# leggedrobotics/delora

Measured on AMD Instinct MI355X. Metric: training scan-pairs/sec, KITTI 64x2048 range images, higher is better.
Workload: dtype f32; 1 GPU; KITTI-shaped 64x2048, batch=8 pairs/GPU, raw scans of ~141k points (ragged, raster order), steps rotate over 8 distinct HBM-resident batches, online normals, ResNet pose CNN (11.9M params, identity-pretrained state), Adam; BASELINE configs[1]; global_batch=8, parallelism=dp1, cnn=fp32, cnn_impl=hip trunk: fp32 MFMA, fused Winograd F(2x2,3x3) + direct implicit GEMM, channels_last=False, hip_graph=False, distinct_batches=8, priming_steps=8

## Files before the change

delora_amd/_lib.py:

```python
import ctypes
import os

_HERE = os.path.dirname(os.path.abspath(__file__))
LIB_PATH = os.path.join(_HERE, "csrc", "libdelora_hip.so")
ABI_VERSION = 10


class DeloraHipError(RuntimeError):
    pass


class SensorStruct(ctypes.Structure):
    _fields_ = [("H", ctypes.c_int32), ("W", ctypes.c_int32),
                ("hfov0", ctypes.c_double), ("hfov1", ctypes.c_double),
                ("vfov0", ctypes.c_double), ("vfov1", ctypes.c_double)]


class RecordLayout(ctypes.Structure):
    _fields_ = [("point_step", ctypes.c_int32), ("off_x", ctypes.c_int32), ("off_y", ctypes.c_int32), ("off_z", ctypes.c_int32),
                ("filter", ctypes.c_uint32), ("min_range", ctypes.c_float)]


RECORDS_DROP_ZERO, RECORDS_MIN_RANGE = 1, 2

# ... 48 lines not shown
    "dl_tower_conv3x3_nhwc_f32": (_i32, [_vp, _vp, _vp, _vp, _i32, _i32, _i32, _i32, _i32, _vp, _vp, _vp, _i32, _i32, _u32, _vp]),
    "dl_tower_wgrad_workspace_bytes": (_sz, [_i32, _i32, _i32, _i32, _i32]),
    "dl_tower_wgrad3x3_nhwc_f32": (_i32, [_vp, _vp, _vp, _vp, _i32, _i32, _i32, _i32, _i32, _vp, _vp, _vp]),
    "dl_narrow_conv2d_nhwc_f32": (_i32, [_vp, _vp, _vp, _vp, _vp, _i32, _i32, _i32, _i32, _i32, _i32, _i32, _i32, _i32, _i32, _u32, _vp]),
    "dl_narrow_dgrad_strided_nhwc_f32": (_i32, [_vp, _vp, _vp, _vp, _vp, _i32, _i32, _i32, _i32, _i32, _i32, _i32, _i32, _i32, _i32, _u32, _vp]),
    "dl_narrow_wgrad_workspace_bytes": (_sz, [_i32, _i32, _i32, _i32, _i32, _i32, _i32, _i32]),
    "dl_narrow_wgrad_nhwc_f32": (_i32, [_vp, _vp, _vp, _vp, _i32, _i32, _i32, _i32, _i32, _i32, _i32, _i32, _vp]),
    "dl_wino_weights_floats": (_sz, [_i32, _i32]),
    "dl_wino_weights_f32": (_i32, [_vp, _vp, _vp, _i32, _i32, _vp]),
    "dl_wino_weights_batch_f32": (_i32, [_vp, _i32, _vp]),
    "dl_wino_conv3x3_workspace_bytes": (_sz, [_i32, _i32, _i32, _i32, _i32]),
    "dl_wino_conv3x3_nhwc_f32": (_i32, [_vp, _vp, _vp, _vp, _vp, _i32, _i32, _i32, _i32, _i32, _i32, _u32, _vp, _vp]),
    "dl_wino_strided_takes": (_i32, [_i32, _i32, _i32, _i32, _i32, _i32, _i32, _i32]),
    "dl_wino_strided_weights_floats": (_sz, [_i32, _i32, _i32, _i32]),
    "dl_wino_strided_weights_f32": (_i32, [_vp, _vp, _vp, _i32, _i32, _i32, _i32, _vp]),
    "dl_wino_strided_conv3x3_nhwc_f32": (_i32, [_vp, _vp, _vp, _i32, _i32, _i32, _i32, _i32, _i32, _i32, _i32, _u32, _vp]),
    "dl_wino_strided_dgrad3x3_nhwc_f32": (_i32, [_vp, _vp, _vp, _vp, _vp, _i32, _i32, _i32, _i32, _i32, _i32, _i32, _i32, _u32, _vp]),
    "dl_wino_wgrad_workspace_bytes": (_sz, [_i32, _i32, _i32, _i32, _i32]),
    "dl_wino_wgrad3x3_nhwc_f32": (_i32, [_vp, _vp, _vp, _vp, _i32, _i32, _i32, _i32, _i32, _vp]),
    "dl_pool3x3s12_nhwc_fwd": (_i32, [_vp, _i32, _i32, _i32, _i32, _vp, _vp, _vp]),
    "dl_pool3x3s12_nhwc_bwd": (_i32, [_vp, _vp, _vp, _i32, _i32, _i32, _i32, _i32, _vp, _vp]),
    "dl_stem_wgrad_workspace_bytes": (_sz, [_i32, _i32, _i32]),
    "dl_stem_wgrad_f32": (_i32, [_vp, _vp, _vp, _vp, _i32, _i32, _i32, _i32, _vp, _vp, _vp]),
    "dl_quat_to_T_fwd": (_i32, [_vp, _vp, _i32, ctypes.c_float, _vp, _vp]),
    "dl_quat_to_T_bwd": (_i32, [_vp, _vp, _i32, ctypes.c_float, _vp, _vp, _vp]),
    "dl_mean_hw_nhwc_f32": (_i32, [_vp, _i32, _i32, _i32, _vp, _vp]),
    "dl_conv_weights_h": (_i32, [_vp, _vp, _vp, _i32, _i32, _i32, _i32, _vp]),
    "dl_conv_weights_batch_h": (_i32, [_vp, _i32, _i32, _vp]),
    "dl_conv2d_nhwc_h": (_i32, [_vp, _vp, _vp, _vp, _vp, _i32, _i32, _i32, _i32, _i32, _i32, _i32, _i32, _i32, _i32, _i32, _u32, _vp]),
    "dl_conv2d_dgrad_strided_nhwc_h": (_i32, [_vp, _vp, _vp, _vp, _vp, _i32, _i32, _i32, _i32, _i32, _i32, _i32, _i32, _i32, _i32, _i32,
                                              _u32, _vp, _vp]),
    "dl_cast_f32_to_h": (_i32, [_vp, _vp, _i64, _i32, _vp]),
    "dl_heads_fwd": (_i32, [_vp, _vp, _i32, _i32, _i32, _i32, _i32, _vp, _vp, _vp, _vp, _vp, _vp, _vp]),
    "dl_heads_bwd_workspace_bytes": (_sz, [_i32, _i32, _i32, _i32]),
    "dl_heads_bwd": (_i32, [_vp, _vp, _i32, _i32, _i32, _i32, _i32, _vp, _vp, _vp, _vp, _vp, _vp, _vp, _vp, _vp, _vp]),
    "dl_heads_fwd_drop": (_i32, [_vp, _vp, _i32, _i32, _i32, _i32, _i32, _vp, _vp, _vp, _vp, _vp, _vp, _vp, _vp]),
    "dl_heads_bwd_drop": (_i32, [_vp, _vp, _i32, _i32, _i32, _i32, _i32, _vp, _vp, _vp, _vp, _vp, _vp, _vp, _vp, _vp, _vp, _vp]),
    "dl_heads_single_fwd": (_i32, [_vp, _vp, _i32, _i32, _i32, _i32, _i32, _i32, _i32, _i32, _vp, _vp, _vp, _vp, _vp, _vp, _vp]),
    "dl_heads_single_bwd_workspace_bytes": (_sz, [_i32, _i32, _i32, _i32, _i32, _i32, _i32]),
    "dl_heads_single_bwd": (_i32, [_vp, _vp, _i32, _i32, _i32, _i32, _i32, _i32, _i32, _i32, _vp, _vp, _vp, _vp, _vp, _vp, _vp, _vp, _vp, _vp]),
    "dl_dropout_scale_f32": (_i32, [_vp, _u32, ctypes.c_double, _i64, _vp, _vp]),
    "dl_stem_input_nhwc_drop_f32": (_i32, [_vp, _i32, _i32, _i32, _i32, _vp, ctypes.c_double, _vp, _vp]),
    "dl_channel_scale_nhwc_t": (_i32, [_vp, _vp, _i32, _i32, _i32, _i32, _vp, _vp]),
    "dl_channel_scale_bwd_act_nhwc_t": (_i32, [_vp, _vp, _vp, _i32, _i32, _i32, _i32, _i32, _vp, _vp]),
    "dl_tower_wide_drop_f32": (_i32, [_vp, _vp, ctypes.c_double, _i32, _i32, _i32, _i32, _i32, _vp, _vp]),
    "dl_tower_wide_drop_bwd_f32": (_i32, [_vp, _vp, _vp, ctypes.c_double, _i32, _i32, _i32, _i32, _i32, _i32, _vp, _vp]),
# ... 135 lines not shown
```

delora_amd/csrc/infer.hip:

```cpp
#include <stdint.h>
#include <stdio.h>
#include <string.h>

#include "common.h"

typedef uint32_t u32x4i __attribute__((ext_vector_type(4)));

__global__ __launch_bounds__(DL_BLOCK) void k_interleave_pair(const uint32_t* __restrict__ prev, size_t prev_ss, const uint32_t* __restrict__ cur,
                                                              size_t cur_ss, uint32_t HW, uint32_t total, u32x4i* __restrict__ x8) {
  const uint32_t i = blockIdx.x * DL_BLOCK + threadIdx.x;
  if (i >= total) return;
  const uint32_t b = i / HW, p = i - b * HW;
  const uint32_t* a = prev + (size_t)b * prev_ss + p;
  const uint32_t* c = cur + (size_t)b * cur_ss + p;
  const u32x4i lo = {a[0], a[HW], a[2 * (size_t)HW], a[3 * (size_t)HW]};
  const u32x4i hi = {c[0], c[HW], c[2 * (size_t)HW], c[3 * (size_t)HW]};
  x8[2 * (size_t)i] = lo;
  x8[2 * (size_t)i + 1] = hi;
}

__global__ void k_single_scan_offsets(int32_t* __restrict__ offs, int32_t n) {
  if (threadIdx.x < 2) offs[threadIdx.x] = threadIdx.x ? n : 0;
}

// ... 97 lines not shown
}

int at_layer(const char* who, const char* what, int block, int rc) {
  if (!rc) return DL_OK;
  char inner[160];
  snprintf(inner, sizeof(inner), "%s", g_dl_err);
  if (block >= 0) return dl_fail(rc, "%s: blocks[%d].%s: %s", who, block, what, inner);
  return dl_fail(rc, "%s: %s: %s", who, what, inner);
}

int pose_forward(const char* who, const dl_pose_net* net, const PosePlan& p, const void* prepared, const float* image_prev, int64_t prev_ss,
                 const float* image_cur, int64_t cur_ss, int B, int H, int W, void* workspace, float* translation, float* quaternion, float* T,
                 dl_stream stream) {
  char* const ws = (char*)workspace;
  float* slot[4];
  for (int i = 0; i < 4; ++i) slot[i] = (float*)(ws + p.slot_off[i]);
  void* const split_ws = p.split_bytes ? (void*)(ws + p.split_off) : nullptr;
  const int act = net->act;
  hipStream_t st = (hipStream_t)stream;
  const uint32_t total = (uint32_t)B * H * W;
  hipLaunchKernelGGL(k_interleave_pair, dim3((total + DL_BLOCK - 1) / DL_BLOCK), dim3(DL_BLOCK), 0, st, (const uint32_t*)image_prev, (size_t)prev_ss,
                     (const uint32_t*)image_cur, (size_t)cur_ss, (uint32_t)(H * W), total, (u32x4i*)slot[0]);
  if (int rc = dl_check_launch(who)) return rc;
  if (int rc = at_layer(who, "conv1", -1, dl_conv2d_nhwc_f32(slot[0], net->conv1_w, slot[1], nullptr, nullptr, B, H, W, 8, 64, 3, 1, 2, 0, act, DL_CONV_ACT, stream)))
    return rc;
  if (int rc = at_layer(who, "pooling", -1, dl_pool3x3s12_nhwc_fwd(slot[1], B, H, W / 2, 64, slot[2], (int8_t*)(ws + p.win_off), stream))) return rc;
  const float* u = (const float*)prepared;
  int s = 2, h = H, w = W / 4;
  for (int i = 0; i < net->n_blocks; ++i) {
    const dl_pose_block& b = net->blocks[i];
    const int ho = ceil_div(h, b.stride_h), wo = ceil_div(w, b.stride_w);
    const float* x = slot[s];
    float *y1 = slot[(s + 1) & 3], *sc = slot[(s + 2) & 3], *y2 = slot[(s + 3) & 3];
    int rc;
    if (runs_wino(b.stride_h, b.stride_w)) {
      rc = dl_wino_conv3x3_nhwc_f32(x, u, y1, nullptr, nullptr, B, h, w, b.cin, b.cout, act, DL_CONV_ACT, split_ws, stream);
      u += dl_wino_weights_floats(b.cout, b.cin);
    } else {
      rc = dl_conv2d_nhwc_f32(x, b.w1, y1, nullptr, nullptr, B, h, w, b.cin, b.cout, 3, b.stride_h, b.stride_w, 0, act, DL_CONV_ACT, stream);
    }
    if ((rc = at_layer(who, "w1", i, rc))) return rc;
    const float* shortcut = x;
    if (b.has_downsample) {
      if ((rc = at_layer(who, "wd", i, dl_conv2d_nhwc_f32(x, b.wd, sc, nullptr, nullptr, B, h, w, b.cin, b.cout, 1, b.stride_h, b.stride_w, 0, 0, 0, stream))))
        return rc;
      shortcut = sc;
    }
// ... 139 lines not shown
```

delora_amd/csrc/stem.hip:

```cpp
#include "common.h"

#define ST_TANH 1
#define ST_RELU 2

typedef float f32x4s __attribute__((ext_vector_type(4)));

__global__ __launch_bounds__(DL_BLOCK) void k_pool_nhwc_fwd(const float* __restrict__ a, int H, int Wc, int C4, uint32_t total,
                                                            float* __restrict__ y, int8_t* __restrict__ win) {
  const uint32_t i = blockIdx.x * DL_BLOCK + threadIdx.x;
  if (i >= total) return;
  const int Wp = Wc >> 1;
  const uint32_t pix = i / (uint32_t)C4;
  const int c4 = (int)(i - pix * (uint32_t)C4);
  const uint32_t nr = pix / (uint32_t)Wp;
  const int q = (int)(pix - nr * (uint32_t)Wp);
  const int r = (int)(nr % (uint32_t)H);
  const int first = r > 0 ? 0 : 3;
  f32x4s best = {-INFINITY, -INFINITY, -INFINITY, -INFINITY};
  int k0 = first, k1 = first, k2 = first, k3 = first;
#pragma unroll
  for (int dh = -1; dh <= 1; ++dh) {
    if (r + dh < 0 || r + dh >= H) continue;
    const float* row = a + ((size_t)(nr + dh) * Wc) * (size_t)(4 * C4) + 4 * c4;
#pragma unroll
    for (int dw = -1; dw <= 1; ++dw) {
      int j = 2 * q + dw;
      j = j < 0 ? j + Wc : j;
      const f32x4s v = *reinterpret_cast<const f32x4s*>(row + (size_t)j * (4 * C4));
      const int k = (dh + 1) * 3 + dw + 1;
      if (v.x > best.x || v.x != v.x) { best.x = v.x; k0 = k; }
      if (v.y > best.y || v.y != v.y) { best.y = v.y; k1 = k; }
      if (v.z > best.z || v.z != v.z) { best.z = v.z; k2 = k; }
      if (v.w > best.w || v.w != v.w) { best.w = v.w; k3 = k; }
    }
  }
  *reinterpret_cast<f32x4s*>(y + (size_t)i * 4) = best;
  *reinterpret_cast<uint32_t*>(win + (size_t)i * 4) = (uint32_t)k0 | ((uint32_t)k1 << 8) | ((uint32_t)k2 << 16) | ((uint32_t)k3 << 24);
}

__device__ __forceinline__ f32x4s pool_bwd_value(const float* __restrict__ g, const float* __restrict__ a, const int8_t* __restrict__ win,
                                                 int H, int Wc, int C4, int act, uint32_t nr, int r, int j, int c4) {
  const int Wp = Wc >> 1;
  const int q0 = j >> 1, col0 = 1 + (j & 1);
  const int q1 = (q0 + 1 == Wp) ? 0 : q0 + 1;
  const bool two = (j & 1) != 0;
  uint32_t w4[6];
  f32x4s gv[6];
  uint32_t code[6];
#pragma unroll
  for (int d = -1; d <= 1; ++d) {
    const bool row_ok = r + d >= 0 && r + d < H;
    const size_t rowbase = (size_t)(nr + (row_ok ? d : 0)) * Wp;
#pragma unroll
    for (int t = 0; t < 2; ++t) {
      const int i = (d + 1) * 2 + t;
      const size_t e = ((rowbase + ((t && two) ? q1 : q0)) * (size_t)C4 + c4) * 4;
      w4[i] = *reinterpret_cast<const uint32_t*>(win + e);
      gv[i] = *reinterpret_cast<const f32x4s*>(g + e);
      code[i] = (row_ok && (t == 0 || two)) ? (uint32_t)((1 - d) * 3 + (t ? 0 : col0)) : 0xffu;
    }
  }
  f32x4s acc = {0.f, 0.f, 0.f, 0.f};
#pragma unroll
  for (int i = 0; i < 6; ++i) {
    acc.x += (w4[i] & 0xffu) == code[i] ? gv[i].x : 0.f;
    acc.y += ((w4[i] >> 8) & 0xffu) == code[i] ? gv[i].y : 0.f;
    acc.z += ((w4[i] >> 16) & 0xffu) == code[i] ? gv[i].z : 0.f;
    acc.w += (w4[i] >> 24) == code[i] ? gv[i].w : 0.f;
  }
  const f32x4s av = *reinterpret_cast<const f32x4s*>(a + (((size_t)nr * Wc + j) * C4 + c4) * 4);
  f32x4s out;
  if (act == ST_TANH) {
    out.x = acc.x * (1.f - av.x * av.x); out.y = acc.y * (1.f - av.y * av.y);
    out.z = acc.z * (1.f - av.z * av.z); out.w = acc.w * (1.f - av.w * av.w);
  } else if (act == ST_RELU) {
    out.x = av.x <= 0.f ? 0.f : acc.x; out.y = av.y <= 0.f ? 0.f : acc.y;
    out.z = av.z <= 0.f ? 0.f : acc.z; out.w = av.w <= 0.f ? 0.f : acc.w;
  } else {
    out = acc;
  }
  return out;
}

__global__ __launch_bounds__(DL_BLOCK) void k_pool_nhwc_bwd(const float* __restrict__ g, const float* __restrict__ a,
                                                            const int8_t* __restrict__ win, int H, int Wc, int C4, int act,
                                                            uint32_t total, float* __restrict__ g_conv) {
  const uint32_t i = blockIdx.x * DL_BLOCK + threadIdx.x;
  if (i >= total) return;
  const uint32_t pix = i / (uint32_t)C4;
  const int c4 = (int)(i - pix * (uint32_t)C4);
  const uint32_t nr = pix / (uint32_t)Wc;
  const int j = (int)(pix - nr * (uint32_t)Wc);
  const int r = (int)(nr % (uint32_t)H);
  *reinterpret_cast<f32x4s*>(g_conv + (size_t)i * 4) = pool_bwd_value(g, a, win, H, Wc, C4, act, nr, r, j, c4);
}

#define SG_PX 64
#define SG_XCOLS (2 * SG_PX + 2)
typedef float f32x16s __attribute__((ext_vector_type(16)));

__global__ __launch_bounds__(DL_BLOCK, 2) void k_stem_wgrad(const float* __restrict__ g, const float* __restrict__ a,
                                                            const int8_t* __restrict__ win, const float* __restrict__ x8, int N, int H,
                                                            int Wc, int act, int chunks_per_slab, float* __restrict__ part) {
  constexpr int K = 64, C4 = 16;
  __shared__ __attribute__((aligned(16))) float gc[SG_PX * K];
  __shared__ __attribute__((aligned(16))) float xt[3 * SG_XCOLS * 8];
  const int tid = threadIdx.x, lane = tid & 63, wave = tid >> 6;
  const int li = lane & 31, half = lane >> 5;
  const int W = 2 * Wc;
  const int cpr = (Wc + SG_PX - 1) / SG_PX;
  const int total = N * H * cpr;
  const int ch_begin = blockIdx.x * chunks_per_slab, ch_end = min(ch_begin + chunks_per_slab, total);
  f32x16s acc[2][3];
#pragma unroll
  for (int i = 0; i < 2; ++i)
#pragma unroll
    for (int j = 0; j < 3; ++j)
#pragma unroll
      for (int r = 0; r < 16; ++r) acc[i][j][r] = 0.f;
  int b_off[3];
#pragma unroll
  for (int ns = 0; ns < 3; ++ns) {
    const int j = min(li + 32 * ns, 71), tap = j >> 3, c = j & 7;
    b_off[ns] = ((tap / 3) * SG_XCOLS + (tap % 3)) * 8 + c;
  }
  for (int ch = ch_begin; ch < ch_end; ++ch) {
    const int cb = ch % cpr;
    const uint32_t nr = (uint32_t)(ch / cpr);
    const int h = (int)(nr % (uint32_t)H), wc0 = cb * SG_PX;
    __syncthreads();
#pragma unroll
    for (int it = 0; it < SG_PX * C4 / DL_BLOCK; ++it) {
      const int q = tid + it * DL_BLOCK, pl = q / C4, c4 = q % C4;
      f32x4s v = {0.f, 0.f, 0.f, 0.f};
      if (wc0 + pl < Wc) v = pool_bwd_value(g, a, win, H, Wc, C4, act, nr, h, wc0 + pl, c4);
      *reinterpret_cast<f32x4s*>(gc + pl * K + c4 * 4) = v;
    }
    for (int q = tid; q < 3 * SG_XCOLS * 2; q += DL_BLOCK) {
      const int hp = q & 1, col = (q >> 1) % SG_XCOLS, row = (q >> 1) / SG_XCOLS;
      const int hh = h + row - 1;
      int w = (2 * wc0 - 1 + col) % W;
      w = w < 0 ? w + W : w;
      f32x4s v = {0.f, 0.f, 0.f, 0.f};
      if (hh >= 0 && hh < H) v = *reinterpret_cast<const f32x4s*>(x8 + (((size_t)(nr + row - 1)) * W + w) * 8 + hp * 4);
      *reinterpret_cast<f32x4s*>(xt + (row * SG_XCOLS + col) * 8 + hp * 4) = v;
    }
    __syncthreads();
#pragma unroll
    for (int ks = 0; ks < 8; ++ks) {
      const int pl = wave * 16 + ks * 2 + half;
      const float a0 = gc[pl * K + li], a1 = gc[pl * K + 32 + li];
      float b[3];
#pragma unroll
      for (int ns = 0; ns < 3; ++ns) b[ns] = xt[b_off[ns] + 2 * pl * 8];
#pragma unroll
      for (int ns = 0; ns < 3; ++ns) {
        acc[0][ns] = __builtin_amdgcn_mfma_f32_32x32x2f32(a0, b[ns], acc[0][ns], 0, 0, 0);
        acc[1][ns] = __builtin_amdgcn_mfma_f32_32x32x2f32(a1, b[ns], acc[1][ns], 0, 0, 0);
      }
    }
  }
  __syncthreads();
  float* red = gc;
#pragma unroll
  for (int ms = 0; ms < 2; ++ms)
#pragma unroll
    for (int ns = 0; ns < 3; ++ns) {
      if (wave > 0)
#pragma unroll
        for (int r = 0; r < 16; ++r) red[(wave - 1) * 1024 + r * 64 + lane] = acc[ms][ns][r];
      __syncthreads();
      if (wave == 0) {
#pragma unroll
        for (int r = 0; r < 16; ++r) acc[ms][ns][r] = ((acc[ms][ns][r] + red[r * 64 + lane]) + red[1024 + r * 64 + lane]) + red[2048 + r * 64 + lane];
        const int j = ns * 32 + li;
        if (j < 72)
#pragma unroll
          for (int r = 0; r < 16; ++r) {
            const int k = ms * 32 + (r & 3) + 8 * (r >> 2) + 4 * half;
            part[((size_t)blockIdx.x * K + k) * 72 + j] = acc[ms][ns][r];
          }
      }
      __syncthreads();
    }
}

__global__ __launch_bounds__(DL_BLOCK) void k_stem_wgrad_reduce(const float* __restrict__ part, int nslabs, float* __restrict__ dw) {
  __shared__ float red[4][64];
  const int i = blockIdx.x * 64 + (threadIdx.x & 63), w = threadIdx.x >> 6;
  float s = 0.f;
  int sl = w;
  for (; sl + 28 < nslabs; sl += 32) {
    float v[8];
#pragma unroll
    for (int u = 0; u < 8; ++u) v[u] = part[(size_t)(sl + 4 * u) * 64 * 72 + i];
#pragma unroll
    for (int u = 0; u < 8; ++u) s += v[u];
  }
  for (; sl < nslabs; sl += 4) s += part[(size_t)sl * 64 * 72 + i];
  red[w][threadIdx.x & 63] = s;
  __syncthreads();
  if (w == 0) {
    const float t = ((red[0][threadIdx.x] + red[1][threadIdx.x]) + red[2][threadIdx.x]) + red[3][threadIdx.x];
// ... 61 lines not shown

static int stem_wgrad_slabs(int total_chunks) { return total_chunks < 512 ? total_chunks : 512; }

extern "C" size_t dl_stem_wgrad_workspace_bytes(int32_t N, int32_t H, int32_t W) {
  if (N <= 0 || H <= 0 || W <= 0 || W % 4) return 0;
  return (size_t)stem_wgrad_slabs(N * H * ((W / 2 + SG_PX - 1) / SG_PX)) * 64 * 72 * sizeof(float);
}

extern "C" int dl_stem_wgrad_f32(const float* g_pooled, const float* a, const int8_t* win, const float* x8, int32_t N, int32_t H,
                                 int32_t W, int32_t act, void* workspace, float* dw, dl_stream stream) {
  if (!g_pooled || !a || !win || !x8 || !workspace || !dw || N <= 0 || H <= 0 || W <= 0 || act < 0 || act > 2)
    return dl_fail(DL_ERR_INVALID_ARGUMENT, "dl_stem_wgrad_f32: bad argument");
  if (W % 4 || (size_t)N * H * W * 32 >= ((size_t)1 << 32))
    return dl_fail(DL_ERR_UNSUPPORTED, "dl_stem_wgrad_f32: N=%d H=%d W=%d not supported (W %% 4, conv1 output below 2^32 elements)", N, H, W);
  const int Wc = W / 2, total = N * H * ((Wc + SG_PX - 1) / SG_PX), nslabs = stem_wgrad_slabs(total);
  const int cps = (total + nslabs - 1) / nslabs, grid = (total + cps - 1) / cps;
  hipStream_t st = (hipStream_t)stream;
  const DlProfTag tag{"k_stem_wgrad", "wgrad", N, H, W, 8, 64, 3, 1, 2, 2.0 * N * H * Wc * 64.0 * 72.0,
                      4.0 * ((double)N * H * Wc * 64 * 1.5 + (double)N * H * W * 8) + (double)N * H * (Wc / 2) * 64};
  DL_LAUNCH(tag, k_stem_wgrad, dim3(grid), dim3(DL_BLOCK), st, g_pooled, a, win, x8, N, H, Wc, act, cps, (float*)workspace);
  hipLaunchKernelGGL(k_stem_wgrad_reduce, dim3(64 * 72 / 64), dim3(DL_BLOCK), 0, st, (const float*)workspace, grid, dw);
  return dl_check_launch("dl_stem_wgrad_f32");
}
```

delora_amd/models/ring_conv.py:

```python
import ctypes
import os

import torch

from .. import _lib

ACT = {"none": 0, "tanh": 1, "relu": 2}
USE_WINOGRAD = True
EPI_ADD, EPI_ACT, EPI_DACT, EPI_ADD_GRID = 1, 2, 4, 8


def _ptr(t):
    return ctypes.c_void_p(t.data_ptr()) if t is not None else ctypes.c_void_p(0)


def _stream():
    return ctypes.c_void_p(torch.cuda.current_stream().cuda_stream)


ALLOC_SKEW = 0
_skew_state = {"i": 0}


def _empty(shape, dtype, device):
# ... 13 lines not shown
    return v if v.is_contiguous() else v.contiguous()


def grad_for(dw_krsc, w_param):
    shape, stride = (tuple(w_param.shape), tuple(w_param.stride())) if torch.is_tensor(w_param) else w_param
    g = dw_krsc.permute(0, 3, 1, 2)
    if tuple(g.stride()) != stride and shape[2] == 1 and shape[3] == 1 and stride[0] == shape[1] and stride[1] == 1:
        g = g.as_strided(shape, stride)
    return g


def out_size(n, stride):
    return -(-int(n) // int(stride))


def conv_nhwc(x, w_krsc, stride=(1, 1), act=0, epilogue=0, add=None, dsrc=None, transposed=False):
    lib = _lib.load()
    N, H, W, C = x.shape
    ks = w_krsc.shape[1]
    K = w_krsc.shape[3] if transposed else w_krsc.shape[0]
    y = _empty((N, out_size(H, stride[0]), out_size(W, stride[1]), K), torch.float32, x.device)
    _lib.check(lib.dl_conv2d_nhwc_f32(_ptr(x), _ptr(w_krsc), _ptr(y), _ptr(add), _ptr(dsrc), N, H, W, C, K, ks, stride[0],
                                      stride[1], int(transposed), int(act), int(epilogue), _stream()), "dl_conv2d_nhwc_f32")
    return y


USE_WINOGRAD_WGRAD = True


def wgrad_nhwc(x, g, ks, stride=(1, 1)):
    lib = _lib.load()
    N, H, W, C = x.shape
    K = g.shape[3]
    dw = torch.empty((K, ks, ks, C), dtype=torch.float32, device=x.device)
    if USE_WINOGRAD_WGRAD and ks == 3 and tuple(stride) == (1, 1) and C >= 128:
        nbytes = lib.dl_wino_wgrad_workspace_bytes(N, H, W, C, K)
        if nbytes:
            ws = torch.empty((nbytes // 4,), dtype=torch.float32, device=x.device)
            _lib.check(lib.dl_wino_wgrad3x3_nhwc_f32(_ptr(x), _ptr(g), _ptr(dw), _ptr(ws), N, H, W, C, K, _stream()),
                       "dl_wino_wgrad3x3_nhwc_f32")
            return dw
    ws = torch.empty((lib.dl_conv2d_wgrad_workspace_bytes(N, H, W, C, K, ks, stride[0], stride[1]) // 4,), dtype=torch.float32,
                     device=x.device)
    _lib.check(lib.dl_conv2d_wgrad_nhwc_f32(_ptr(x), _ptr(g), _ptr(dw), _ptr(ws), N, H, W, C, K, ks, stride[0], stride[1],
                                            _stream()), "dl_conv2d_wgrad_nhwc_f32")
    return dw
# ... 332 lines not shown

def stem_supported(x_shape, out_channels):
    N, C, H, W = x_shape
    k_ok = out_channels % 64 == 0 or (C == 8 and out_channels in NARROW_STEM_CHANNELS and N * H * W * 64 < (1 << 31))
    return ((C % 8 == 0 and C % 16 != 0) or C == TOWER_CHANNELS) and k_ok and W % 4 == 0 and W >= 4 and H >= 1


def planar_stem_supported(x_shape, out_channels):
    return stem_supported(x_shape, out_channels) and x_shape[1] % 16 != 0


class RingStem(torch.autograd.Function):

    @staticmethod
    def forward(ctx, x, w1, act, *drop):
        if drop and drop[0] is not None:
            seed, p = drop[0]
            x8 = stem_input_drop(x, seed, p)
            ctx.drop_p = float(p)
        else:
            seed = None
            x8 = x.permute(0, 2, 3, 1).contiguous()
        ctx.n_extra = len(drop)
        conv1 = conv_nhwc if w1.shape[0] % 64 == 0 else narrow_conv
        a = conv1(x8, weight_storage(w1), stride=(1, 2), act=act, epilogue=EPI_ACT if act else 0)
        y, win = pool_fwd(a)
        ctx.save_for_backward(x8, a, win, w1, *([seed] if seed is not None else []))
        ctx.act = act
        return y

    @staticmethod
    def backward(ctx, g):
        x8, a, win, w1, *seed = ctx.saved_tensors
        extra = (None,) * ctx.n_extra
        want_x = ctx.needs_input_grad[0]
        lib = _lib.load()
        N, H, W, _ = x8.shape
        nbytes = 0 if want_x or a.shape[3] != 64 or x8.shape[3] != 8 else lib.dl_stem_wgrad_workspace_bytes(N, H, W)
        if nbytes:
            ws = torch.empty((nbytes // 4,), dtype=torch.float32, device=x8.device)
            dw = torch.empty((64, 8, 3, 3), dtype=torch.float32, device=x8.device)
            _lib.check(lib.dl_stem_wgrad_f32(_ptr(g.contiguous()), _ptr(a), _ptr(win), _ptr(x8), N, H, W, int(ctx.act), _ptr(ws), _ptr(dw),
                                             _stream()), "dl_stem_wgrad_f32")
            return (None, dw, None) + extra
        gc = pool_bwd(g.contiguous(), a, win, ctx.act)
        if not want_x and a.shape[3] % 64:
            dw = narrow_wgrad(x8, gc, 3, stride=(1, 2)).permute(0, 3, 1, 2)
            return (None, dw if tuple(dw.stride()) == tuple(w1.stride()) else dw.contiguous(), None) + extra
# ... 614 lines not shown
```

include/delora_hip.h:

```cpp
#ifndef DELORA_HIP_H
#define DELORA_HIP_H

#include <stddef.h>
#include <stdint.h>

#ifdef __cplusplus
extern "C" {
#endif

#define DL_ABI_VERSION 10

typedef void* dl_stream;

typedef enum {
  DL_OK = 0,
  DL_ERR_INVALID_ARGUMENT = -1,
  DL_ERR_LAUNCH = -2,
  DL_ERR_UNSUPPORTED = -3
} dl_status;

typedef struct {
  int32_t H;
  int32_t W;
  double hfov0, hfov1;
// ... 204 lines not shown
                                   int32_t H, int32_t W, int32_t K, int32_t C, int32_t ksize, int32_t stride_h, int32_t stride_w,
                                   int32_t dense, int32_t dtype, int32_t act, uint32_t epilogue, float* seam_ws, dl_stream stream);
int dl_cast_f32_to_h(const float* src, void* dst, int64_t n, int32_t dtype, dl_stream stream);
int dl_mean_hw_nhwc_h(const void* x, int32_t N, int32_t P, int32_t C, int32_t dtype, float* y, dl_stream stream);
int dl_mean_hw_bwd_act_h(const float* grad_y, const void* x, int32_t N, int32_t P, int32_t C, int32_t act, int32_t dtype,
                         void* grad_pre, dl_stream stream);
size_t dl_conv2d_wgrad_h_workspace_bytes(int32_t N, int32_t H, int32_t W, int32_t C, int32_t K, int32_t ksize, int32_t stride_h,
                                         int32_t stride_w);
int dl_conv2d_wgrad_nhwc_h(const void* x, const void* g, float* dw, void* workspace, int32_t N, int32_t H, int32_t W, int32_t C,
                           int32_t K, int32_t ksize, int32_t stride_h, int32_t stride_w, int32_t dtype, dl_stream stream);

typedef dl_wgrad_layer dl_wgrad_h_layer;
size_t dl_conv2d_wgrad_batch_h_workspace_bytes(const dl_wgrad_h_layer* layers, int32_t n);
int dl_conv2d_wgrad_batch_nhwc_h(const dl_wgrad_h_layer* layers, int32_t n, void* workspace, int32_t dtype, dl_stream stream);

int dl_pool3x3s12_nhwc_fwd(const float* a, int32_t N, int32_t H, int32_t W, int32_t C, float* y, int8_t* win, dl_stream stream);
int dl_pool3x3s12_nhwc_bwd(const float* g, const float* a, const int8_t* win, int32_t N, int32_t H, int32_t W, int32_t C,
                           int32_t act, float* g_conv, dl_stream stream);

size_t dl_stem_wgrad_workspace_bytes(int32_t N, int32_t H, int32_t W);
int dl_stem_wgrad_f32(const float* g_pooled, const float* a, const int8_t* win, const float* x8, int32_t N, int32_t H, int32_t W,
                      int32_t act, void* workspace, float* dw, dl_stream stream);

typedef struct {
  const float *fc_w, *fc_b;
  const float *r1_w, *r1_b;
  const float *r3_w, *r3_b;
  const float *t1_w, *t1_b;
  const float *t3_w, *t3_b;
} dl_heads_params;
int dl_heads_fwd(const float* x, const dl_heads_params* params, int32_t B, int32_t F, int32_t R, int32_t Hd, int32_t act, float* a1,
                 float* a2, float* rot_raw, float* translation, float* rotation, float* norm, dl_stream stream);
size_t dl_heads_bwd_workspace_bytes(int32_t B, int32_t F, int32_t R, int32_t Hd);
int dl_heads_bwd(const float* x, const dl_heads_params* params, int32_t B, int32_t F, int32_t R, int32_t Hd, int32_t act, const float* a1,
                 const float* a2, const float* rot_raw, const float* norm, const float* grad_translation, const float* grad_rotation,
                 const dl_heads_params* grads, float* grad_x, void* workspace, dl_stream stream);

int dl_heads_fwd_drop(const float* x, const dl_heads_params* params, int32_t B, int32_t F, int32_t R, int32_t Hd, int32_t act,
                      const float* fc_scale, float* a1, float* a2, float* rot_raw, float* translation, float* rotation, float* norm,
                      dl_stream stream);
int dl_heads_bwd_drop(const float* x, const dl_heads_params* params, int32_t B, int32_t F, int32_t R, int32_t Hd, int32_t act,
                      const float* fc_scale, const float* a1, const float* a2, const float* rot_raw, const float* norm,
                      const float* grad_translation, const float* grad_rotation, const dl_heads_params* grads, float* grad_x,
                      void* workspace, dl_stream stream);

typedef struct {
// ... 85 lines not shown
```

Baseline: 684.1 scan-pairs/s.

## Add dedicated stem conv1 MFMA kernel and software-pipeline stem wgrad staging

Adds a specialised forward kernel for the 8-to-64-channel stride-(1,2) stem convolution. It keeps the weights in registers, runs one tile per wave with register prefetch of the next tile, and applies the activation in the epilogue. It replaces the generic NHWC conv in both the training and inference paths. The stem weight-gradient kernel now prefetches the next chunk's pooled gradients, window codes, activations and inputs into registers and double-buffers them in LDS, and it uses an XCD-aware block swizzle. This overlaps global loads with MFMA work, at the cost of more registers and LDS, and adds ablation macros.

```diff
diff --git a/delora_amd/_lib.py b/delora_amd/_lib.py
--- a/delora_amd/_lib.py
+++ b/delora_amd/_lib.py
@@ -94,6 +94,7 @@
     "dl_pool3x3s12_nhwc_bwd": (_i32, [_vp, _vp, _vp, _i32, _i32, _i32, _i32, _i32, _vp, _vp]),
     "dl_stem_wgrad_workspace_bytes": (_sz, [_i32, _i32, _i32]),
     "dl_stem_wgrad_f32": (_i32, [_vp, _vp, _vp, _vp, _i32, _i32, _i32, _i32, _vp, _vp, _vp]),
+    "dl_stem_conv1_f32": (_i32, [_vp, _vp, _vp, _i32, _i32, _i32, _i32, _vp]),
     "dl_quat_to_T_fwd": (_i32, [_vp, _vp, _i32, ctypes.c_float, _vp, _vp]),
     "dl_quat_to_T_bwd": (_i32, [_vp, _vp, _i32, ctypes.c_float, _vp, _vp, _vp]),
     "dl_mean_hw_nhwc_f32": (_i32, [_vp, _i32, _i32, _i32, _vp, _vp]),
diff --git a/delora_amd/csrc/infer.hip b/delora_amd/csrc/infer.hip
--- a/delora_amd/csrc/infer.hip
+++ b/delora_amd/csrc/infer.hip
@@ -143,7 +143,7 @@
   hipLaunchKernelGGL(k_interleave_pair, dim3((total + DL_BLOCK - 1) / DL_BLOCK), dim3(DL_BLOCK), 0, st, (const uint32_t*)image_prev, (size_t)prev_ss,
                      (const uint32_t*)image_cur, (size_t)cur_ss, (uint32_t)(H * W), total, (u32x4i*)slot[0]);
   if (int rc = dl_check_launch(who)) return rc;
-  if (int rc = at_layer(who, "conv1", -1, dl_conv2d_nhwc_f32(slot[0], net->conv1_w, slot[1], nullptr, nullptr, B, H, W, 8, 64, 3, 1, 2, 0, act, DL_CONV_ACT, stream)))
+  if (int rc = at_layer(who, "conv1", -1, dl_stem_conv1_f32(slot[0], net->conv1_w, slot[1], B, H, W, act, stream)))
     return rc;
   if (int rc = at_layer(who, "pooling", -1, dl_pool3x3s12_nhwc_fwd(slot[1], B, H, W / 2, 64, slot[2], (int8_t*)(ws + p.win_off), stream))) return rc;
   const float* u = (const float*)prepared;
diff --git a/delora_amd/csrc/stem.hip b/delora_amd/csrc/stem.hip
--- a/delora_amd/csrc/stem.hip
+++ b/delora_amd/csrc/stem.hip
@@ -1,5 +1,8 @@
 #include "common.h"
 
+#ifndef ST_ABL
+#define ST_ABL 0
+#endif
 #define ST_TANH 1
 #define ST_RELU 2
 
@@ -38,6 +41,29 @@
   *reinterpret_cast<uint32_t*>(win + (size_t)i * 4) = (uint32_t)k0 | ((uint32_t)k1 << 8) | ((uint32_t)k2 << 16) | ((uint32_t)k3 << 24);
 }
 
+template <int NC>
+__device__ __forceinline__ f32x4s pool_bwd_combine(const uint32_t (&w4)[NC], const f32x4s (&gv)[NC], const uint32_t (&code)[NC], f32x4s av, int act) {
+  f32x4s acc = {0.f, 0.f, 0.f, 0.f};
+#pragma unroll
+  for (int i = 0; i < NC; ++i) {
+    acc.x += (w4[i] & 0xffu) == code[i] ? gv[i].x : 0.f;
+    acc.y += ((w4[i] >> 8) & 0xffu) == code[i] ? gv[i].y : 0.f;
+    acc.z += ((w4[i] >> 16) & 0xffu) == code[i] ? gv[i].z : 0.f;
+    acc.w += (w4[i] >> 24) == code[i] ? gv[i].w : 0.f;
+  }
+  f32x4s out;
+  if (act == ST_TANH) {
+    out.x = acc.x * (1.f - av.x * av.x); out.y = acc.y * (1.f - av.y * av.y);
+    out.z = acc.z * (1.f - av.z * av.z); out.w = acc.w * (1.f - av.w * av.w);
+  } else if (act == ST_RELU) {
+    out.x = av.x <= 0.f ? 0.f : acc.x; out.y = av.y <= 0.f ? 0.f : acc.y;
+    out.z = av.z <= 0.f ? 0.f : acc.z; out.w = av.w <= 0.f ? 0.f : acc.w;
+  } else {
+    out = acc;
+  }
+  return out;
+}
+
 __device__ __forceinline__ f32x4s pool_bwd_value(const float* __restrict__ g, const float* __restrict__ a, const int8_t* __restrict__ win,
                                                  int H, int Wc, int C4, int act, uint32_t nr, int r, int j, int c4) {
   const int Wp = Wc >> 1;
@@ -60,26 +86,8 @@
       code[i] = (row_ok && (t == 0 || two)) ? (uint32_t)((1 - d) * 3 + (t ? 0 : col0)) : 0xffu;
     }
   }
-  f32x4s acc = {0.f, 0.f, 0.f, 0.f};
-#pragma unroll
-  for (int i = 0; i < 6; ++i) {
-    acc.x += (w4[i] & 0xffu) == code[i] ? gv[i].x : 0.f;
-    acc.y += ((w4[i] >> 8) & 0xffu) == code[i] ? gv[i].y : 0.f;
-    acc.z += ((w4[i] >> 16) & 0xffu) == code[i] ? gv[i].z : 0.f;
-    acc.w += (w4[i] >> 24) == code[i] ? gv[i].w : 0.f;
-  }
   const f32x4s av = *reinterpret_cast<const f32x4s*>(a + (((size_t)nr * Wc + j) * C4 + c4) * 4);
-  f32x4s out;
-  if (act == ST_TANH) {
-    out.x = acc.x * (1.f - av.x * av.x); out.y = acc.y * (1.f - av.y * av.y);
-    out.z = acc.z * (1.f - av.z * av.z); out.w = acc.w * (1.f - av.w * av.w);
-  } else if (act == ST_RELU) {
-    out.x = av.x <= 0.f ? 0.f : acc.x; out.y = av.y <= 0.f ? 0.f : acc.y;
-    out.z = av.z <= 0.f ? 0.f : acc.z; out.w = av.w <= 0.f ? 0.f : acc.w;
-  } else {
-    out = acc;
-  }
-  return out;
+  return pool_bwd_combine<6>(w4, gv, code, av, act);
 }
 
 __global__ __launch_bounds__(DL_BLOCK) void k_pool_nhwc_bwd(const float* __restrict__ g, const float* __restrict__ a,
@@ -97,20 +105,34 @@
 
 #define SG_PX 64
 #define SG_XCOLS (2 * SG_PX + 2)
+#define SG_NQ (SG_PX / 2 + 1)
+#define SG_GITEMS (3 * SG_NQ * 16)
+#define SG_XITEMS (3 * SG_XCOLS * 2)
+#define SG_GIT ((SG_GITEMS + DL_BLOCK - 1) / DL_BLOCK)
+#define SG_XIT ((SG_XITEMS + DL_BLOCK - 1) / DL_BLOCK)
+#define SG_AIT (SG_PX * 16 / DL_BLOCK)
 typedef float f32x16s __attribute__((ext_vector_type(16)));
+
+__device__ __forceinline__ int sg_xcd_swizzle(int id, int n) {
+  const int q = n / 8, r = n % 8, xcd = id % 8, k = id / 8;
+  return (xcd < r ? xcd * (q + 1) : r * (q + 1) + (xcd - r) * q) + k;
+}
 
 __global__ __launch_bounds__(DL_BLOCK, 2) void k_stem_wgrad(const float* __restrict__ g, const float* __restrict__ a,
                                                             const int8_t* __restrict__ win, const float* __restrict__ x8, int N, int H,
                                                             int Wc, int act, int chunks_per_slab, float* __restrict__ part) {
-  constexpr int K = 64, C4 = 16;
+  constexpr int K = 64;
   __shared__ __attribute__((aligned(16))) float gc[SG_PX * K];
-  __shared__ __attribute__((aligned(16))) float xt[3 * SG_XCOLS * 8];
+  __shared__ __attribute__((aligned(16))) float xt[2][3 * SG_XCOLS * 8];
+  __shared__ __attribute__((aligned(16))) float sg[SG_GITEMS * 4];
+  __shared__ uint32_t sw[SG_GITEMS];
   const int tid = threadIdx.x, lane = tid & 63, wave = tid >> 6;
   const int li = lane & 31, half = lane >> 5;
-  const int W = 2 * Wc;
+  const int W = 2 * Wc, Wp = Wc >> 1;
   const int cpr = (Wc + SG_PX - 1) / SG_PX;
   const int total = N * H * cpr;
-  const int ch_begin = blockIdx.x * chunks_per_slab, ch_end = min(ch_begin + chunks_per_slab, total);
+  const int slab = sg_xcd_swizzle(blockIdx.x, gridDim.x);
+  const int ch_begin = slab * chunks_per_slab, ch_end = min(ch_begin + chunks_per_slab, total);
   f32x16s acc[2][3];
 #pragma unroll
   for (int i = 0; i < 2; ++i)
@@ -124,42 +146,136 @@
     const int j = min(li + 32 * ns, 71), tap = j >> 3, c = j & 7;
     b_off[ns] = ((tap / 3) * SG_XCOLS + (tap % 3)) * 8 + c;
   }
+  f32x4s rg[SG_GIT], ra[SG_AIT], rx[SG_XIT];
+  uint32_t rw[SG_GIT];
+#define SG_FETCH(CH)                                                                                                      \
+  {                                                                                                                       \
+    const int cb_ = (CH) % cpr;                                                                                           \
+    const uint32_t nr_ = (uint32_t)((CH) / cpr);                                                           \
+    const int h_ = (int)(nr_ % (uint32_t)H), wc0_ = cb_ * SG_PX;                                                          \
+    int t_ = tid;                                                                                                         \
+    asm volatile("" : "+v"(t_));                                                                                          \
+     \
+    const size_t gr_ = ((size_t)nr_ - 1) * (size_t)Wp * 64;                                                               \
+    const float* gb_ = g + gr_;                                                                                           \
+    const int8_t* wb_ = win + gr_;                                                                                        \
+    const float* ab_ = a + (size_t)nr_ * (size_t)Wc * 64;                                                                 \
+    const float* xb_ = x8 + ((size_t)nr_ - 1) * (size_t)W * 8;                                                            \
+    _Pragma("unroll") for (int it = 0; it < SG_GIT; ++it) {                                                               \
+      const int q = min(t_ + it * DL_BLOCK, SG_GITEMS - 1), c4 = q & 15, ps = q >> 4, row = ps / SG_NQ, s = ps - row * SG_NQ; \
+      const int hh = h_ + row - 1;                                                                                        \
+      const int rr = (hh >= 0 && hh < H) ? row : 1;                                     \
+      int col = (wc0_ >> 1) + s;                                                                                          \
+      col = col >= Wp ? 0 : col;                                    \
+      const uint32_t e = (uint32_t)((rr * Wp + col) * 16 + c4) * 4u;                                                      \
+      rg[it] = (ST_ABL & 16) ? (f32x4s){(float)e, 1.f, 2.f, 3.f} : *reinterpret_cast<const f32x4s*>((const char*)gb_ + 4u * e);            \
+      rw[it] = (ST_ABL & 16) ? e : *reinterpret_cast<const uint32_t*>(wb_ + e);                                           \
+    }                                                                                                                     \
+    _Pragma("unroll") for (int it = 0; it < SG_AIT; ++it) {                                                               \
+      const int pl = 2 * ((t_ >> 4) + (it & 1) * 16) + (it >> 1), c4 = t_ & 15;       \
+      const uint32_t ea = (uint32_t)(min(wc0_ + pl, Wc - 1) * 16 + c4) * 4u;                                              \
+      ra[it] = (ST_ABL & 16) ? (f32x4s){(float)ea, 1.f, 2.f, 3.f} : *reinterpret_cast<const f32x4s*>((const char*)ab_ + 4u * ea);          \
+    }                                                                                                                     \
+    _Pragma("unroll") for (int it = 0; it < SG_XIT; ++it) {                                                               \
+      const int q = min(t_ + it * DL_BLOCK, SG_XITEMS - 1), hp = q & 1, pc = q >> 1, row = pc / SG_XCOLS, col = pc - row * SG_XCOLS; \
+      const int hh = h_ + row - 1;                                                                                        \
+      const bool ok = hh >= 0 && hh < H;                                                                                  \
+      int w = 2 * wc0_ - 1 + col;                                                        \
+      w = w < 0 ? w + W : w;                                                                                              \
+      w = w >= W ? w - W : w;                                                                                             \
+      if (W < 2 * SG_PX) w %= W;                                    \
+      const uint32_t ex = (uint32_t)(((ok ? row : 1) * W + w) * 8 + hp * 4);                                              \
+      const f32x4s v = (ST_ABL & 16) ? (f32x4s){(float)ex, 1.f, 2.f, 3.f} : *reinterpret_cast<const f32x4s*>((const char*)xb_ + 4u * ex);  \
+      rx[it] = ok ? v : (f32x4s){0.f, 0.f, 0.f, 0.f};                                                                     \
+    }                                                                                                                     \
+  }
+#define SG_STAGE(BUF)                                                                                                     \
+  {                                                                                                                       \
+    int t_ = tid;                                                                                                         \
+    asm volatile("" : "+v"(t_));                                                                                          \
+    _Pragma("unroll") for (int it = 0; it < SG_GIT; ++it) {                                                               \
+      const int q = min(t_ + it * DL_BLOCK, SG_GITEMS - 1);                                                              \
+      *reinterpret_cast<f32x4s*>(sg + q * 4) = rg[it];                                                                    \
+      sw[q] = rw[it];                                                                                                     \
+    }                                                                                                                     \
+    _Pragma("unroll") for (int it = 0; it < SG_XIT; ++it)                                                                 \
+      *reinterpret_cast<f32x4s*>(xt[BUF] + min(t_ + it * DL_BLOCK, SG_XITEMS - 1) * 4) = rx[it];                         \
+  }
+  if (ch_begin < ch_end) {
+    SG_FETCH(ch_begin)
+    SG_STAGE(0)
+  }
   for (int ch = ch_begin; ch < ch_end; ++ch) {
+    const int buf = (ch - ch_begin) & 1;
     const int cb = ch % cpr;
-    const uint32_t nr = (uint32_t)(ch / cpr);
-    const int h = (int)(nr % (uint32_t)H), wc0 = cb * SG_PX;
+    const int h = (int)((uint32_t)(ch / cpr) % (uint32_t)H), wc0 = cb * SG_PX;
     __syncthreads();
-#pragma unroll
-    for (int it = 0; it < SG_PX * C4 / DL_BLOCK; ++it) {
-      const int q = tid + it * DL_BLOCK, pl = q / C4, c4 = q % C4;
-      f32x4s v = {0.f, 0.f, 0.f, 0.f};
-      if (wc0 + pl < Wc) v = pool_bwd_value(g, a, win, H, Wc, C4, act, nr, h, wc0 + pl, c4);
+    int tb = tid;
+    asm volatile("" : "+v"(tb));
+    static_assert(SG_AIT == 4, "two iterations per column parity");
+#pragma unroll
+    for (int it = 0; it < ((ST_ABL & 32) ? 0 : SG_AIT); ++it) {
+      const int s0 = (tb >> 4) + (it & 1) * 16, pl = 2 * s0 + (it >> 1), c4 = tb & 15;
+      f32x4s v;
+      if (it < 2) {
+        uint32_t w4[3], code[3];
+        f32x4s gv[3];
+#pragma unroll
+        for (int d = -1; d <= 1; ++d) {
+          const int e = ((d + 1) * SG_NQ + s0) * 16 + c4;
+          w4[d + 1] = sw[e];
+          gv[d + 1] = *reinterpret_cast<const f32x4s*>(sg + e * 4);
+          code[d + 1] = (h + d >= 0 && h + d < H) ? (uint32_t)((1 - d) * 3 + 1) : 0xffu;
+        }
+        v = pool_bwd_combine<3>(w4, gv, code, ra[it], act);
+      } else {
+        uint32_t w4[6], code[6];
+        f32x4s gv[6];
+#pragma unroll
+        for (int d = -1; d <= 1; ++d) {
+          const bool row_ok = h + d >= 0 && h + d < H;
+#pragma unroll
+          for (int t = 0; t < 2; ++t) {
+            const int i = (d + 1) * 2 + t, e = ((d + 1) * SG_NQ + s0 + t) * 16 + c4;
+            w4[i] = sw[e];
+            gv[i] = *reinterpret_cast<const f32x4s*>(sg + e * 4);
+            code[i] = row_ok ? (uint32_t)((1 - d) * 3 + (t ? 0 : 2)) : 0xffu;
+          }
+        }
+        v = pool_bwd_combine<6>(w4, gv, code, ra[it], act);
+      }
+      if (wc0 + pl >= Wc) v = (f32x4s){0.f, 0.f, 0.f, 0.f};
       *reinterpret_cast<f32x4s*>(gc + pl * K + c4 * 4) = v;
-    }
-    for (int q = tid; q < 3 * SG_XCOLS * 2; q += DL_BLOCK) {
-      const int hp = q & 1, col = (q >> 1) % SG_XCOLS, row = (q >> 1) / SG_XCOLS;
-      const int hh = h + row - 1;
-      int w = (2 * wc0 - 1 + col) % W;
-      w = w < 0 ? w + W : w;
-      f32x4s v = {0.f, 0.f, 0.f, 0.f};
-      if (hh >= 0 && hh < H) v = *reinterpret_cast<const f32x4s*>(x8 + (((size_t)(nr + row - 1)) * W + w) * 8 + hp * 4);
-      *reinterpret_cast<f32x4s*>(xt + (row * SG_XCOLS + col) * 8 + hp * 4) = v;
+      __builtin_amdgcn_sched_barrier(0);
     }
     __syncthreads();
+    const int nxt = min(ch + 1, ch_end - 1);
+    SG_FETCH(nxt)
+    __builtin_amdgcn_sched_barrier(0);
+    const float* xc = xt[buf];
 #pragma unroll
     for (int ks = 0; ks < 8; ++ks) {
       const int pl = wave * 16 + ks * 2 + half;
       const float a0 = gc[pl * K + li], a1 = gc[pl * K + 32 + li];
       float b[3];
 #pragma unroll
-      for (int ns = 0; ns < 3; ++ns) b[ns] = xt[b_off[ns] + 2 * pl * 8];
+      for (int ns = 0; ns < 3; ++ns) b[ns] = xc[b_off[ns] + 2 * pl * 8];
 #pragma unroll
       for (int ns = 0; ns < 3; ++ns) {
+#if ST_ABL & 8
+        acc[0][ns][ks] += a0 * b[ns];
+        acc[1][ns][ks] += a1 * b[ns];
+#else
         acc[0][ns] = __builtin_amdgcn_mfma_f32_32x32x2f32(a0, b[ns], acc[0][ns], 0, 0, 0);
         acc[1][ns] = __builtin_amdgcn_mfma_f32_32x32x2f32(a1, b[ns], acc[1][ns], 0, 0, 0);
+#endif
       }
     }
-  }
+    __builtin_amdgcn_sched_barrier(0);
+    SG_STAGE(buf ^ 1)
+  }
+#undef SG_FETCH
+#undef SG_STAGE
   __syncthreads();
   float* red = gc;
 #pragma unroll
@@ -178,7 +294,7 @@
 #pragma unroll
           for (int r = 0; r < 16; ++r) {
             const int k = ms * 32 + (r & 3) + 8 * (r >> 2) + 4 * half;
-            part[((size_t)blockIdx.x * K + k) * 72 + j] = acc[ms][ns][r];
+            part[((size_t)slab * K + k) * 72 + j] = acc[ms][ns][r];
           }
       }
       __syncthreads();
@@ -286,3 +402,126 @@
   hipLaunchKernelGGL(k_stem_wgrad_reduce, dim3(64 * 72 / 64), dim3(DL_BLOCK), 0, st, (const float*)workspace, grid, dw);
   return dl_check_launch("dl_stem_wgrad_f32");
 }
+
+#define C1_PX 32
+#define C1_COLS (2 * C1_PX + 1)
+#define C1_S 12
+#define C1_XITEMS (3 * C1_COLS * 2)
+#define C1_XIT ((C1_XITEMS + 63) / 64)
+#define C1_ES 68
+#define C1_WAVE_FLOATS (3 * C1_COLS * C1_S + C1_PX * C1_ES)
+
+__device__ __forceinline__ float st_act(float v, int act) {
+  if (act == ST_TANH) return dl_tanh(v);
+  if (act == ST_RELU) return v < 0.f ? 0.f : v;
+  return v;
+}
+
+__global__ __launch_bounds__(DL_BLOCK, 2) void k_stem_conv1(const float* __restrict__ x8, const float* __restrict__ w, float* __restrict__ y,
+                                                            int H, int W, int act, int ntiles) {
+  __shared__ __attribute__((aligned(16))) float lds[4 * C1_WAVE_FLOATS];
+  const int lane = threadIdx.x & 63, wave = threadIdx.x >> 6, li = lane & 31, half = lane >> 5;
+  float* xp = lds + wave * C1_WAVE_FLOATS;
+  float* ep = xp + 3 * C1_COLS * C1_S;
+  const int Wc = W >> 1, tpr = (Wc + C1_PX - 1) / C1_PX;
+  f32x4s bw[9][2];
+#pragma unroll
+  for (int tap = 0; tap < 9; ++tap)
+#pragma unroll
+    for (int ni = 0; ni < 2; ++ni) bw[tap][ni] = *reinterpret_cast<const f32x4s*>(w + ((ni * 32 + li) * 9 + tap) * 8 + half * 4);
+  const int wg = sg_xcd_swizzle(blockIdx.x, gridDim.x), stride = gridDim.x * 4;
+  f32x4s rx[C1_XIT];
+#define C1_FETCH(T)                                                                                                       \
+  {                                                                                                                       \
+    const uint32_t nr_ = (uint32_t)((T) / tpr);                                                            \
+    const int h_ = (int)(nr_ % (uint32_t)H), w0_ = 2 * C1_PX * ((T) % tpr) - 1;                                           \
+    int l_ = lane;                                                                                                        \
+    asm volatile("" : "+v"(l_));                                        \
+    const float* xb_ = x8 + ((size_t)nr_ - 1) * (size_t)W * 8;          \
+    _Pragma("unroll") for (int it = 0; it < C1_XIT; ++it) {                                                               \
+      const int q = min(l_ + it * 64, C1_XITEMS - 1), hp = q & 1, pc = q >> 1, row = pc / C1_COLS, col = pc - row * C1_COLS; \
+      const int hh = h_ + row - 1;                                                                                        \
+      int ww = w0_ + col;                                                                                                 \
+      ww = ww < 0 ? ww + W : ww;                                                                                          \
+       \
+      const bool ok = hh >= 0 && hh < H && ww < W;                                                                        \
+      const uint32_t e = (uint32_t)(((ok ? row : 1) * W + (ok ? ww : 0)) * 8 + hp * 4);                                   \
+      const f32x4s v = (ST_ABL & 4) ? (f32x4s){(float)e, 1.f, 2.f, 3.f} : *reinterpret_cast<const f32x4s*>((const char*)xb_ + 4u * e);    \
+      rx[it] = ok ? v : (f32x4s){0.f, 0.f, 0.f, 0.f};                                                                     \
+    }                                                                                                                     \
+  }
+#define C1_STAGE()                                                                                                        \
+  {                                                                                                                       \
+    int l_ = lane;                                                                                                        \
+    asm volatile("" : "+v"(l_));                                                                                          \
+    _Pragma("unroll") for (int it = 0; it < C1_XIT; ++it) {                                                               \
+      const int q = min(l_ + it * 64, C1_XITEMS - 1);                                                                     \
+      *reinterpret_cast<f32x4s*>(xp + (q >> 1) * C1_S + (q & 1) * 4) = rx[it];                                            \
+    }                                                                                                                     \
+  }
+  int t = wg * 4 + wave;
+  if (t < ntiles) {
+    C1_FETCH(t)
+    C1_STAGE()
+  }
+  const int a_off = 2 * li * C1_S + half * 4;
+  for (; t < ntiles; t += stride) {
+    const int tn = t + stride < ntiles ? t + stride : t;
+    C1_FETCH(tn)
+    __builtin_amdgcn_sched_barrier(0);
+    f32x16s acc[2];
+#pragma unroll
+    for (int ni = 0; ni < 2; ++ni)
+#pragma unroll
+      for (int r = 0; r < 16; ++r) acc[ni][r] = 0.f;
+#pragma unroll
+    for (int tap = 0; tap < 9; ++tap) {
+      const f32x4s af = *reinterpret_cast<const f32x4s*>(xp + a_off + ((tap / 3) * C1_COLS + tap % 3) * C1_S);
+#pragma unroll
+      for (int j = 0; j < 4; ++j)
+#pragma unroll
+        for (int ni = 0; ni < 2; ++ni)
+#if ST_ABL & 1
+          acc[ni][j] += af[j] * bw[tap][ni][j];
+#else
+          acc[ni] = __builtin_amdgcn_mfma_f32_32x32x2f32(af[j], bw[tap][ni][j], acc[ni], 0, 0, 0);
+#endif
+    }
+#pragma unroll
+    for (int ni = 0; ni < 2; ++ni)
+#pragma unroll
+      for (int r = 0; r < 16; ++r) ep[((r & 3) + 8 * (r >> 2) + 4 * half) * C1_ES + ni * 32 + li] = acc[ni][r];
+    const int wo0 = C1_PX * (t % tpr);
+    float* yb = y + ((size_t)(t / tpr) * Wc + wo0) * 64;
+#pragma unroll 2
+    for (int q = lane; q < C1_PX * 16; q += 64) {
+      const int row = q >> 4, c4 = q & 15;
+      if (wo0 + row >= Wc) continue;
+      f32x4s v = *reinterpret_cast<const f32x4s*>(ep + row * C1_ES + c4 * 4);
+      v.x = st_act(v.x, act); v.y = st_act(v.y, act); v.z = st_act(v.z, act); v.w = st_act(v.w, act);
+#if ST_ABL & 2
+      if (act == 99)
+#endif
+      *reinterpret_cast<f32x4s*>((char*)yb + (uint32_t)(q * 16)) = v;
+    }
+    __builtin_amdgcn_sched_barrier(0);
+    C1_STAGE()
+  }
+#undef C1_FETCH
+#undef C1_STAGE
+}
+
+extern "C" int dl_stem_conv1_f32(const float* x8, const float* w, float* y, int32_t N, int32_t H, int32_t W, int32_t act, dl_stream stream) {
+  if (!x8 || !w || !y || N <= 0 || H <= 0 || W <= 0 || act < 0 || act > 2)
+    return dl_fail(DL_ERR_INVALID_ARGUMENT, "dl_stem_conv1_f32: bad argument");
+  if (((uintptr_t)x8 | (uintptr_t)w | (uintptr_t)y) & 15)
+    return dl_fail(DL_ERR_INVALID_ARGUMENT, "dl_stem_conv1_f32: x8, w and y must be 16-byte aligned");
+  if (W % 4 || (size_t)N * H * W * 8 >= ((size_t)1 << 31) || (size_t)N * H * (W / 2) * 64 >= ((size_t)1 << 31))
+    return dl_fail(DL_ERR_UNSUPPORTED, "dl_stem_conv1_f32: N=%d H=%d W=%d not supported (W %% 4, tensors below 2^31 elements)", N, H, W);
+  const int Wc = W / 2, ntiles = N * H * ((Wc + C1_PX - 1) / C1_PX);
+  const int grid = (ntiles + 3) / 4 < 512 ? (ntiles + 3) / 4 : 512;
+  const DlProfTag tag{"k_stem_conv1", "fwd", N, H, W, 8, 64, 3, 1, 2, 2.0 * N * H * Wc * 64.0 * 72.0,
+                      4.0 * ((double)N * H * W * 8 + (double)N * H * Wc * 64 + 64.0 * 72.0)};
+  DL_LAUNCH(tag, k_stem_conv1, dim3(grid), dim3(DL_BLOCK), (hipStream_t)stream, x8, w, y, H, W, act, ntiles);
+  return dl_check_launch("dl_stem_conv1_f32");
+}
diff --git a/delora_amd/models/ring_conv.py b/delora_amd/models/ring_conv.py
--- a/delora_amd/models/ring_conv.py
+++ b/delora_amd/models/ring_conv.py
@@ -59,6 +59,14 @@
     y = _empty((N, out_size(H, stride[0]), out_size(W, stride[1]), K), torch.float32, x.device)
     _lib.check(lib.dl_conv2d_nhwc_f32(_ptr(x), _ptr(w_krsc), _ptr(y), _ptr(add), _ptr(dsrc), N, H, W, C, K, ks, stride[0],
                                       stride[1], int(transposed), int(act), int(epilogue), _stream()), "dl_conv2d_nhwc_f32")
+    return y
+
+
+def stem_conv1(x8, w_krsc, act=0):
+    lib = _lib.load()
+    N, H, W, _ = x8.shape
+    y = _empty((N, H, W // 2, 64), torch.float32, x8.device)
+    _lib.check(lib.dl_stem_conv1_f32(_ptr(x8), _ptr(w_krsc), _ptr(y), N, H, W, int(act), _stream()), "dl_stem_conv1_f32")
     return y
 
 
@@ -437,8 +445,11 @@
             seed = None
             x8 = x.permute(0, 2, 3, 1).contiguous()
         ctx.n_extra = len(drop)
-        conv1 = conv_nhwc if w1.shape[0] % 64 == 0 else narrow_conv
-        a = conv1(x8, weight_storage(w1), stride=(1, 2), act=act, epilogue=EPI_ACT if act else 0)
+        if w1.shape[0] == 64 and x8.shape[3] == 8:
+            a = stem_conv1(x8, weight_storage(w1), act)
+        else:
+            conv1 = conv_nhwc if w1.shape[0] % 64 == 0 else narrow_conv
+            a = conv1(x8, weight_storage(w1), stride=(1, 2), act=act, epilogue=EPI_ACT if act else 0)
         y, win = pool_fwd(a)
         ctx.save_for_backward(x8, a, win, w1, *([seed] if seed is not None else []))
         ctx.act = act
diff --git a/include/delora_hip.h b/include/delora_hip.h
--- a/include/delora_hip.h
+++ b/include/delora_hip.h
@@ -250,6 +250,8 @@
 int dl_stem_wgrad_f32(const float* g_pooled, const float* a, const int8_t* win, const float* x8, int32_t N, int32_t H, int32_t W,
                       int32_t act, void* workspace, float* dw, dl_stream stream);
 
+int dl_stem_conv1_f32(const float* x8, const float* w, float* y, int32_t N, int32_t H, int32_t W, int32_t act, dl_stream stream);
+
 typedef struct {
   const float *fc_w, *fc_b;
   const float *r1_w, *r1_b;
```

After: 686.3 scan-pairs/s, median of 6. No clear change (+0.3%).
